# david-gimeno/tailored-avsr

Hardware: AMD Instinct MI355X
Metric: utterances/sec fwd+bwd, 12L tailored AV-Branchformer (Conv3d+ResNet-18 lip frontend, fusion, CTC+6L decoder), 4 s clips, batch 32/GPU (higher is better)
Workload: dtype f32

## Files before the change

profiles/conv_launches.py:

```python
import csv
import os
import sys
from collections import defaultdict

ROOT = os.path.dirname(os.path.dirname(os.path.abspath(__file__)))
sys.path[:0] = [ROOT, os.path.join(ROOT, "tailored-avsr_amd")]
N_IMG = 3200
LAYERS = (("layer 4", 3, 3, 512), ("layer 3", 6, 6, 256))
FLAGS = (0, 3, 1)


def labels():
    out = []
    for name, H, W, Cc in LAYERS:
        out += [f"{name} forward NT {N_IMG * H * W}x{Cc}x{9 * Cc} posmajor={f}" for f in FLAGS]
        out += [f"{name} wgrad TN {Cc}x{9 * Cc}x{N_IMG * H * W} posmajor={f}" for f in FLAGS]
    return out


def run():
    import torch
    from tavsr import ops
    for name, H, W, Cc in LAYERS:
        M, K = N_IMG * H * W, 9 * Cc
        x = torch.randn(M, Cc, device="cuda")
        w = torch.randn(Cc, K, device="cuda") / K ** 0.5
        dz = torch.randn(M, Cc, device="cuda")
        z = torch.empty(M, Cc, device="cuda")
        dw = torch.empty(Cc, K, device="cuda")
        for f in FLAGS:
            for _ in range(2):
                ops.gemm(M, Cc, K, x, Cc, w, K, z, Cc, conv=(1, H, W, Cc, 1, 9, f))
        for f in FLAGS:
            for _ in range(2):
                ops.gemm(Cc, K, M, dz, Cc, x, Cc, dw, K, a_kmajor=True, b_kmajor=True, conv=(2, H, W, Cc, 1, 9, f))
        torch.cuda.synchronize()


def summarise(path):
    rows = defaultdict(dict)
    names = {}
    with open(path) as f:
        for r in csv.DictReader(f):
            if "gemm_glds_kernel" not in r["Kernel_Name"]:
                continue
            d = int(r["Dispatch_Id"])
            rows[d][r["Counter_Name"]] = rows[d].get(r["Counter_Name"], 0.0) + float(r["Counter_Value"])
            names[d] = r["Kernel_Name"]
# ... 21 lines not shown
```

tailored-avsr_amd/csrc/gemm.hip:

```cpp
#include <algorithm>
#include <type_traits>
#include <vector>

#include <cstdlib>
#include "common.h"

namespace tavsr {

typedef float f32x16 __attribute__((ext_vector_type(16)));

struct GemmArgs {
  tavsr_gemm_desc d;
  int kchunk;
  int nsplit;
  int tiles_m, tiles_n;
  int vec_epi;
  int zmap;
};

template <int V>
__global__ __launch_bounds__(256) void splitk_epilogue_kernel(const GemmArgs args) {
  const tavsr_gemm_desc& d = args.d;
  const int64_t mn = (int64_t)d.M * d.N;
  const int nbatch = d.nb1 * d.nb2;
  const int64_t i = ((int64_t)blockIdx.x * 256 + threadIdx.x) * V;
  const int z = blockIdx.y, z1 = z / d.nb2, z2 = z % d.nb2;
  if (d.a_rowsum && z == 0 && i < d.M) {
    const float* rs = d.ws + (int64_t)args.nsplit * nbatch * mn;
    for (int q = 0; q < V && i + q < d.M; ++q) {
      float v = 0.f;
      for (int s = 0; s < args.nsplit; ++s) v += rs[(int64_t)s * d.M + i + q];
      d.a_rowsum[i + q] = d.alpha * v;
// ... 128 lines not shown
template <int ROWS, int BK, bool KMAJOR>
__device__ __forceinline__ void read_frag(const float* __restrict__ s, int row, int g, int lk, float (&f)[4]) {
  using T = Tile<ROWS, BK, KMAJOR>;
  if (KMAJOR) {
    const float* p = s + (g * 8 + 4 * lk) * T::LD + row;
#pragma unroll
    for (int j = 0; j < 4; ++j) f[j] = p[j * T::LD];
  } else {
    const float4 v = *reinterpret_cast<const float4*>(s + row * T::LD + g * 8 + 4 * lk);
    f[0] = v.x; f[1] = v.y; f[2] = v.z; f[3] = v.w;
  }
}

struct PosMajor {
  int n, H, W;
  int uni, base, rp;
  __host__ __device__ __forceinline__ void pos(int v, int& y, int& x) const {
    const int Hi = H > 2 ? H - 2 : 0, Wi = W > 2 ? W - 2 : 0, Hb = H - Hi, Wb = W - Wi;
    int u = v;
    if (u < Hi * Wi) { y = u / Wi + 1; x = u % Wi + 1; return; }
    u -= Hi * Wi;
    if (u < Hi * Wb) { y = u / Wb + 1; x = (u % Wb) ? W - 1 : 0; return; }
    u -= Hi * Wb;
    if (u < Hb * Wi) { y = (u / Wi) ? H - 1 : 0; x = u % Wi + 1; return; }
    u -= Hb * Wi;
    y = (u / Wb) ? H - 1 : 0;
    x = (u % Wb) ? W - 1 : 0;
  }
  __host__ __device__ __forceinline__ uint32_t taps(int y, int x) const {
    uint32_t mk = 0;
#pragma unroll
    for (int tap = 0; tap < 9; ++tap)
      mk |= (uint32_t)((unsigned)(y + tap / 3 - 1) < (unsigned)H && (unsigned)(x + tap % 3 - 1) < (unsigned)W) << tap;
    return mk;
  }
  __device__ __forceinline__ int row(int r) const {
    if (uni) return (r - base) * (H * W) + rp;
    const int v = r / n;
    int y, x;
    pos(v, y, x);
    return (r - v * n) * (H * W) + y * W + x;
  }
};

constexpr int kOrdRuns = 80;
struct TileOrder {
  int nruns;
  int start[kOrdRuns];
// ... 14 lines not shown
  }
  const int s = s0 + (uniform ? (j & 7) : j / tiles_n);
  nt = uniform ? (j >> 3) : j % tiles_n;
  int r = r0;
  while (r + 1 < o.nruns && o.cum[r + 1] <= s) ++r;
  mt = o.start[r] + s - o.cum[r];
}

__host__ __device__ inline int dw_tile_order(int q, int tiles_m, int tiles_n, int H, int W) {
  if (tiles_n % 9 != 0) return q;
  const int tpt = tiles_n / 9, per = tiles_m * tpt;
  const int rank = q / per, rem = q - rank * per;
  const unsigned long long taps = (H - 1) * W >= H * (W - 1) ? 0x862053714ull : 0x862071534ull;
  const int tap = (int)((taps >> (4 * rank)) & 15);
  return (rem / tpt) * tiles_n + tap * tpt + rem % tpt;
}

template <int TM, int TN, bool PM = false>
__device__ __forceinline__ void finish_tile(const tavsr_gemm_desc& d, int nsplit, f32x16 (&acc)[TM][TN],
                                            float (&asum)[TM], bool want_rowsum, int m0, int n0, int wm, int wn, int lr,
                                            int lk, int z1, int z2, int64_t coff, int zidx, const float* bias_pre = nullptr,
                                            const PosMajor* pm = nullptr) {
  if (want_rowsum) {
#pragma unroll
    for (int i = 0; i < TM; ++i) asum[i] += __shfl_xor(asum[i], 32, 64);
  }

  if (nsplit > 1) {
    const int64_t mn = (int64_t)d.M * d.N;
    const int nbatch = gridDim.y;
// ... 346 lines not shown
}

#ifdef TAVSR_GEMM_TRACE
constexpr int kTraceMax = 1 << 15;
__device__ unsigned long long g_trace[kTraceMax][6];
__device__ unsigned int g_trace_n;
#define TAVSR_TRACE_DECL unsigned long long tr_t[4], tr_c[4]; tr_t[0] = wall_clock64(); tr_t[1] = tr_t[0]; tr_c[1] = tr_c[2] = 0;
#define TAVSR_TRACE_AT(i) { tr_t[i] = wall_clock64(); tr_c[i] = __builtin_readcyclecounter(); }
#else
#define TAVSR_TRACE_DECL
#define TAVSR_TRACE_AT(i)
#endif

template <int BM, int BN, int WM, int WN, int S, bool AK, bool BKM, int KW = 1, int CONV = 0, bool PM = false>
__device__ __forceinline__ void glds_tile(const tavsr_gemm_desc& d, int kchunk, int nsplit, int tiles_n, int bid, bool vec_epi,
                                          int zidx) {
  constexpr int BK = 32, NG = BK / 8;
  static_assert(NG % KW == 0, "k-groups must divide over the wave sets");
  constexpr int NT = WM * WN * KW * 64;
  constexpr int TM = BM / WM / 32, TN = BN / WN / 32;
  using LA = GLoader<BM, AK, NT>;
  using LB = GLoader<BN, BKM, NT>;
  constexpr int ASZ = BM * BK, STAGE = (BM + BN) * BK;
  constexpr int NR4A = BM * BK / NT, NR4B = BN * BK / NT;
  constexpr int G = (CONV == 4 ? NR4A : LA::NR) + (CONV == 5 ? NR4B : LB::NR);
  static_assert((S - 2) * G <= 63, "vmcnt field");
  static_assert(!PM || (KW == 1 && ((CONV == 1 && !AK) || (CONV == 2 && AK && BKM))), "position-major order: the 3x3 convolution's GEMMs");
  __shared__ __attribute__((aligned(1024))) float smem[S * STAGE];

  const int tid = threadIdx.x;
  const int lane = tid & 63;
// ... 16 lines not shown
#pragma unroll
    for (int j = 0; j < TN; ++j)
#pragma unroll
      for (int r = 0; r < 16; ++r) acc[i][j][r] = 0.f;
  float asum[TM];
#pragma unroll
  for (int i = 0; i < TM; ++i) asum[i] = 0.f;
  const bool want_rowsum = d.a_rowsum != nullptr && n0 == (PM && CONV == 2 ? 4 * d.conv_C : 0) && wn == 0;
  float bpre[TN];
#pragma unroll
  for (int j = 0; j < TN; ++j) {
    const int n = n0 + wn * TN * 32 + j * 32 + lr;
    bpre[j] = (d.bias && nsplit == 1 && n < d.N) ? d.bias[n] : 0.f;
  }

  const int kbeg = zidx * kchunk;
  const int kend = min(d.K, kbeg + kchunk);
  int nk = CONV == 3 ? (kend - kbeg + BK - 1) / BK : (kend - kbeg) / BK;
  const int64_t kstepA = AK ? (int64_t)BK * d.lda : BK;
  const int64_t kstepB = BKM ? (int64_t)BK * d.ldb : BK;
  int64_t offA[LA::NR], offB[LB::NR];
  LA::offsets(d.lda, m0, d.M, tid, offA);
  LB::offsets(d.ldb, n0, d.N, tid, offB);
  const float* Ak = A + (AK ? (int64_t)kbeg * d.lda : kbeg);
  const float* Bk = B + (BKM ? (int64_t)kbeg * d.ldb : kbeg);
  uint32_t cmask[LA::NR];
  const int cs = d.conv_stride > 1 ? d.conv_stride : 1;
  const bool c9 = d.conv_taps != 1;
  const int cp0 = (CONV == 1 || CONV == 2) && d.conv_taps == 90 ? 1 : 0;
  const int cHo = CONV ? (d.conv_H - 1 - 2 * cp0) / cs + 1 : 1, cWo = CONV ? (d.conv_W - 1 - 2 * cp0) / cs + 1 : 1;
  PosMajor pm{};
  uint32_t pm_taps = 0;
  int pm_tap = 0, pm_cb = 0;
  if (PM && CONV == 1) {
    pm.H = d.conv_H; pm.W = d.conv_W;
    pm.n = d.M / (d.conv_H * d.conv_W);
    const int vlo = m0 / pm.n, vhi = min(m0 + BM - 1, d.M - 1) / pm.n;
    for (int v = vlo; v <= vhi; ++v) {
      int y, x;
      pm.pos(v, y, x);
      pm_taps |= pm.taps(y, x);
      pm.rp = y * d.conv_W + x;
    }
    pm.uni = vlo == vhi;
    pm.base = vlo * pm.n;
    nk = 0;
    for (int tap = 0; tap < 9; ++tap) {
      const int lo = max(kbeg, tap * d.conv_C), hi = min(kend, (tap + 1) * d.conv_C);
      if (((pm_taps >> tap) & 1u) && hi > lo) nk += (hi - lo) / BK;
    }
    pm_tap = kbeg / d.conv_C;
    pm_cb = (kbeg - pm_tap * d.conv_C) / BK;
    if (!((pm_taps >> pm_tap) & 1u)) {
      const uint32_t up = pm_taps >> (pm_tap + 1) << (pm_tap + 1);
      pm_tap = up ? __builtin_ctz(up) : 9;
      pm_cb = 0;
    }
#pragma unroll
    for (int i = 0; i < LA::NR; ++i) {
      const int q = i * NT + tid, row = q >> 3;
      const int r = min(m0 + row, d.M - 1);
      int y, x, img;
      if (pm.uni) {
        y = pm.rp / d.conv_W; x = pm.rp - y * d.conv_W; img = r - pm.base;
      } else {
        const int v = r / pm.n;
        pm.pos(v, y, x);
        img = r - v * pm.n;
      }
      offA[i] = ((int64_t)img * (d.conv_H * d.conv_W) + y * d.conv_W + x) * d.lda + ((q & 7) ^ ((row >> 1) & 7)) * 4;
      cmask[i] = pm.taps(y, x);
    }
  } else if (CONV == 1) {
#pragma unroll
    for (int i = 0; i < LA::NR; ++i) {
      const int m = min(m0 + ((i * NT + tid) >> 3), d.M - 1);
      const int x = (m % cWo) * cs + cp0, y = ((m / cWo) % cHo) * cs + cp0;
      if (cs > 1 || cp0) offA[i] += ((int64_t)((m / (cWo * cHo)) * d.conv_H + y) * d.conv_W + x - m) * d.conv_C;
      uint32_t mk = 0;
#pragma unroll
      for (int tap = 0; tap < 9; ++tap)
        mk |= (uint32_t)((unsigned)(y + tap / 3 - 1) < (unsigned)d.conv_H && (unsigned)(x + tap % 3 - 1) < (unsigned)d.conv_W) << tap;
      cmask[i] = c9 ? mk : 1u;
    }
  }
// ... 78 lines not shown
    c2_cb = n0 - tap * d.conv_C;
    c2_dy = c9 ? tap / 3 - 1 : 0;
    c2_dx = c9 ? tap % 3 - 1 : 0;
    c2_tapoff = c2_dy * d.conv_W + c2_dx;
#pragma unroll
    for (int i = 0; i < LB::NR; ++i) {
      const int m = kbeg + (i * NT + tid) / (BN / 4);
      const int t = m / cWo;
      c2_ox[i] = m - t * cWo;
      c2_img[i] = t / cHo;
      c2_oy[i] = t - c2_img[i] * cHo;
    }
  }
  int p2_n = 1, p2_i0 = 0, p2_v = 0, p2_img = 0, p2_x = 0, p2_y = 0;
  auto p2_ok = [&](int y, int x) {
    return (unsigned)(y + c2_dy) < (unsigned)d.conv_H && (unsigned)(x + c2_dx) < (unsigned)d.conv_W;
  };
  auto p2_advance = [&]() {
    p2_img += BK;
    while (p2_img >= p2_n) {
      p2_img -= p2_n;
      ++p2_v;
      if (++p2_x == d.conv_W) { p2_x = 0; ++p2_y; }
    }
  };
  if (PM && CONV == 2) {
    const int P = d.conv_H * d.conv_W;
    p2_i0 = kbeg / P;
    p2_n = (kend - kbeg) / P;
#pragma unroll
    for (int i = 0; i < LA::NR; ++i) offA[i] -= (int64_t)((i * NT + tid) / (BM / 4)) * d.lda;
    if (p2_n % BK == 0) {
      nk = (p2_n / BK) * max(d.conv_H - abs(c2_dy), 0) * max(d.conv_W - abs(c2_dx), 0);
    } else {
      nk = 0;
      int prev = 0, y = 0, x = 0;
      for (int v = 0; v < P; ++v) {
        if (p2_ok(y, x)) {
          const int s_lo = max(v * p2_n / BK, prev), s_hi = ((v + 1) * p2_n - 1) / BK + 1;
          if (s_hi > s_lo) { nk += s_hi - s_lo; prev = s_hi; }
        }
        if (++x == d.conv_W) { x = 0; ++y; }
      }
    }
  }
  int kofsA[LA::NR], kofsB[LB::NR];
  if (CONV == 3) {
#pragma unroll
    for (int i = 0; i < LA::NR; ++i) {
      const int q = i * NT + tid;
      kofsA[i] = AK ? q / (BM / 4) : ((q & 7) ^ (((q >> 3) >> 1) & 7)) * 4;
    }
#pragma unroll
    for (int i = 0; i < LB::NR; ++i) {
      const int q = i * NT + tid;
      kofsB[i] = BKM ? q / (BN / 4) : ((q & 7) ^ (((q >> 3) >> 1) & 7)) * 4;
    }
  }
  auto issue = [&](int kt, int st) {
    if (PM && CONV == 2) {
      for (;;) {
        bool any = false;
        int end = p2_img + BK, y = p2_y, x = p2_x;
        for (;;) {
          any |= p2_ok(y, x);
          if (end <= p2_n) break;
          end -= p2_n;
          if (++x == d.conv_W) { x = 0; ++y; }
        }
        if (any) break;
        p2_advance();
      }
      const int P = d.conv_H * d.conv_W;
      auto locate = [&](int kl, int& y, int& x) {
        int img = p2_img + kl, v = p2_v;
        y = p2_y; x = p2_x;
        while (img >= p2_n) {
          img -= p2_n;
          ++v;
          if (++x == d.conv_W) { x = 0; ++y; }
        }
        return (int64_t)(p2_i0 + img) * P + v;
      };
#pragma unroll
      for (int i = 0; i < LA::NR; ++i) {
        int y, x;
        const int64_t pix = locate((i * NT + tid) / (BM / 4), y, x);
        __builtin_amdgcn_global_load_lds((glb_float*)(A + pix * d.lda + offA[i]), (lds_float*)(smem + st * STAGE + (i * NT + wave * 64) * 4), 16, 0, 0);
      }
#pragma unroll
      for (int i = 0; i < LB::NR; ++i) {
        const int r = (((i * NT + tid) % (BN / 4)) * 4);
        int y, x;
        const int64_t pix = locate((i * NT + tid) / (BN / 4), y, x);
        const float* src = p2_ok(y, x) ? B + (pix + c2_tapoff) * d.conv_C + c2_cb + r : d.conv_zero;
        __builtin_amdgcn_global_load_lds((glb_float*)src, (lds_float*)(smem + st * STAGE + ASZ + (i * NT + wave * 64) * 4), 16, 0, 0);
      }
      p2_advance();
      return;
    }
    int kpm = 0, kpm_tap = 0;
    if (PM) {
      kpm_tap = pm_tap;
      kpm = pm_tap * d.conv_C + pm_cb * BK;
      const int wrap = (pm_cb + 1) * BK >= d.conv_C;
      const uint32_t up = pm_taps >> (pm_tap + 1) << (pm_tap + 1);
      pm_cb = wrap ? 0 : pm_cb + 1;
      pm_tap = !wrap ? pm_tap : up ? __builtin_ctz(up) : 9;
    }
// ... 252 lines not shown

template <int BM, int BN, int WM, int WN, int S, int MINW, bool AK, bool BKM, int KW = 1, int CONV = 0, bool PM = false>
__global__ __launch_bounds__(WM* WN * KW * 64, MINW)
void gemm_glds_kernel(const std::conditional_t<PM && CONV == 1, GemmArgsOrd, GemmArgs> xargs) {
  const GemmArgs& args = common_args(xargs);
  int bid = xcd_remap(blockIdx.x, gridDim.x), zidx = blockIdx.z;
  if constexpr (PM && CONV == 1) {
    if (xargs.ord.nruns > 0) {
      int mt, nt;
      tile_order_map(xargs.ord, blockIdx.x, args.tiles_m, args.tiles_n, mt, nt);
      bid = mt * args.tiles_n + nt;
    }
  }
  if (args.zmap) {
    const int tiles = gridDim.x, l = blockIdx.x + tiles * blockIdx.z, j = l >> 3;
    zidx = (l & 7) + 8 * (j / tiles);
    bid = j % tiles;
    if constexpr (PM && CONV == 2) {
      if (!(args.d.conv_posmajor & 2)) bid = dw_tile_order(bid, args.tiles_m, args.tiles_n, args.d.conv_H, args.d.conv_W);
    }
  }
  glds_tile<BM, BN, WM, WN, S, AK, BKM, KW, CONV, PM>(args.d, args.kchunk, args.nsplit, args.tiles_n, bid, args.vec_epi != 0, zidx);
}

constexpr int kMaxGroup = 12;
struct GroupArgs {
  tavsr_gemm_desc d[kMaxGroup];
  int tile_start[kMaxGroup + 1];
  int tiles_n[kMaxGroup];
  int n;
  int vec_epi;
};

template <int BM, int BN, int WM, int WN, int S, int MINW, bool AK, bool BKM>
__global__ __launch_bounds__(WM* WN * 64, MINW)
void gemm_glds_grouped_kernel(const GroupArgs g) {
  const int bid = xcd_remap(blockIdx.x, gridDim.x);
// ... 120 lines not shown
}

template <int BM, int BN, int WM, int WN, int S, int MINW, int KW = 1>
static int launch_glds(const tavsr_gemm_desc& d, int nsplit, int kchunk, hipStream_t s) {
  GemmArgs a{d, kchunk, nsplit, cdiv(d.M, BM), cdiv(d.N, BN), (int)vec_epi_ok(d)};
  dim3 grid(a.tiles_m * a.tiles_n, d.nb1 * d.nb2, nsplit);
  int rc = launch_layout(d, [&](auto ak, auto bk) {
    hipLaunchKernelGGL((gemm_glds_kernel<BM, BN, WM, WN, S, MINW, decltype(ak)::value, decltype(bk)::value, KW>), grid,
                       dim3(WM * WN * KW * 64), 0, s, a);
    TAVSR_LAUNCH_CHECK();
    return (int)TAVSR_OK;
  });
  return rc ? rc : launch_epilogue(a, s);
}

static bool conv_pm(const tavsr_gemm_desc& d) {
  return d.conv_posmajor && (d.conv_mode == 1 || d.conv_mode == 2) && d.conv_stride <= 1 && (d.conv_taps == 0 || d.conv_taps == 9) &&
         (d.conv_mode == 2 || !d.a_rowsum);
}

static void tile_order_build(const tavsr_gemm_desc& d, int BM, int nsplit, TileOrder& o) {
  o.nruns = 0;
  const int P = d.conv_H * d.conv_W;
  if (nsplit != 1 || (d.conv_posmajor & 2) || P <= 0 || d.M < P) return;
  struct Key { int H, W, M, BM; };
  static thread_local Key last{0, 0, 0, 0};
  static thread_local TileOrder last_o;
  if (last.H == d.conv_H && last.W == d.conv_W && last.M == d.M && last.BM == BM) { o = last_o; return; }
  PosMajor pm{};
  pm.H = d.conv_H; pm.W = d.conv_W; pm.n = d.M / P;
  std::vector<uint32_t> tp(P);
  for (int v = 0; v < P; ++v) {
    int y, x;
    pm.pos(v, y, x);
    tp[v] = pm.taps(y, x);
  }
  struct Run { int start, len, w; };
  std::vector<Run> runs;
  const int tiles_m = cdiv(d.M, BM);
  for (int i = 0; i < tiles_m; ++i) {
    const int vlo = (int)((int64_t)i * BM / pm.n);
    const int vhi = std::min((int)(std::min<int64_t>((int64_t)i * BM + BM - 1, d.M - 1) / pm.n), P - 1);
    uint32_t mk = 0;
    for (int v = vlo; v <= vhi; ++v) mk |= tp[v];
    const int w = __builtin_popcount(mk);
    if (!runs.empty() && runs.back().w == w) ++runs.back().len;
    else runs.push_back(Run{i, 1, w});
    if ((int)runs.size() > kOrdRuns) return;
  }
  std::stable_sort(runs.begin(), runs.end(), [](const Run& a, const Run& b) { return a.w > b.w; });
  int cum = 0;
  for (size_t r = 0; r < runs.size(); ++r) {
    o.start[r] = runs[r].start; o.cum[r] = cum; o.w[r] = runs[r].w;
    cum += runs[r].len;
  }
  o.cum[runs.size()] = cum;
  o.nruns = (int)runs.size();
  last = Key{d.conv_H, d.conv_W, d.M, BM};
  last_o = o;
}

static int launch_conv(const tavsr_gemm_desc& d, int nsplit, int kchunk, hipStream_t s) {
  const int ve = (int)vec_epi_ok(d);
  constexpr int wide = 1;
  constexpr int dw_wide = 1;
  constexpr int zmap_on = 1;
  const int zmap = zmap_on && (d.conv_mode == 2 || d.conv_mode == 5 || d.conv_mode == 7) && nsplit >= 8 && nsplit % 8 == 0;
  if (d.conv_mode == 6 || d.conv_mode == 7) {
    GemmArgs a6{d, kchunk, nsplit, cdiv(d.M, 64), cdiv(d.N, 64), ve, zmap};
    const dim3 grid6(a6.tiles_m * a6.tiles_n, 1, nsplit);
    constexpr int st3 = 2;
    constexpr int tile128 = 0;
    if (d.conv_mode == 6 && tile128) {
      GemmArgs a7{d, kchunk, nsplit, cdiv(d.M, 128), cdiv(d.N, 64), ve, 0};
      hipLaunchKernelGGL((gemm_glds_kernel<128, 64, 2, 2, 2, 3, false, false, 1, 6>), dim3(a7.tiles_m * a7.tiles_n, 1, 1), dim3(256), 0, s, a7);
      TAVSR_LAUNCH_CHECK();
      return TAVSR_OK;
// ... 20 lines not shown
    return launch_epilogue(a4, s);
  }
  const bool pm = conv_pm(d) && d.conv_mode == 1, pm2 = conv_pm(d) && d.conv_mode == 2;
  if (d.conv_mode == 1 && !d.b_kmajor && nsplit == 1 && wide && d.N % 128 == 0) {
    GemmArgs a2{d, kchunk, nsplit, cdiv(d.M, 64), cdiv(d.N, 128), (int)vec_epi_ok(d)};
    if (pm) {
      GemmArgsOrd ao{a2, {}};
      tile_order_build(d, 64, nsplit, ao.ord);
      hipLaunchKernelGGL((gemm_glds_kernel<64, 128, 2, 2, 2, 3, false, false, 1, 1, true>), dim3(a2.tiles_m * a2.tiles_n, 1, 1), dim3(256), 0, s, ao);
    } else
      hipLaunchKernelGGL((gemm_glds_kernel<64, 128, 2, 2, 2, 3, false, false, 1, 1>), dim3(a2.tiles_m * a2.tiles_n, 1, 1), dim3(256), 0, s, a2);
    TAVSR_LAUNCH_CHECK();
    return TAVSR_OK;
  }
  if (d.conv_mode == 2 && dw_wide && d.M % 128 == 0) {
    GemmArgs a2{d, kchunk, nsplit, cdiv(d.M, 128), cdiv(d.N, 64), (int)vec_epi_ok(d), zmap};
    if (pm2)
      hipLaunchKernelGGL((gemm_glds_kernel<128, 64, 2, 2, 2, 3, true, true, 1, 2, true>), dim3(a2.tiles_m * a2.tiles_n, 1, nsplit), dim3(256), 0, s, a2);
    else
      hipLaunchKernelGGL((gemm_glds_kernel<128, 64, 2, 2, 2, 3, true, true, 1, 2>), dim3(a2.tiles_m * a2.tiles_n, 1, nsplit), dim3(256), 0, s, a2);
    TAVSR_LAUNCH_CHECK();
    return launch_epilogue(a2, s);
  }
  GemmArgs a{d, kchunk, nsplit, cdiv(d.M, 64), cdiv(d.N, 64), ve, zmap};
  dim3 grid(a.tiles_m * a.tiles_n, 1, nsplit);
  if (pm) {
    GemmArgsOrd ao{a, {}};
    tile_order_build(d, 64, nsplit, ao.ord);
    if (!d.b_kmajor)
      hipLaunchKernelGGL((gemm_glds_kernel<64, 64, 2, 2, 2, 5, false, false, 1, 1, true>), grid, dim3(256), 0, s, ao);
    else
      hipLaunchKernelGGL((gemm_glds_kernel<64, 64, 2, 2, 2, 5, false, true, 1, 1, true>), grid, dim3(256), 0, s, ao);
  } else if (d.conv_mode == 1 && !d.b_kmajor)
    hipLaunchKernelGGL((gemm_glds_kernel<64, 64, 2, 2, 2, 5, false, false, 1, 1>), grid, dim3(256), 0, s, a);
  else if (d.conv_mode == 1)
    hipLaunchKernelGGL((gemm_glds_kernel<64, 64, 2, 2, 2, 5, false, true, 1, 1>), grid, dim3(256), 0, s, a);
  else if (pm2)
    hipLaunchKernelGGL((gemm_glds_kernel<64, 64, 2, 2, 2, 5, true, true, 1, 2, true>), grid, dim3(256), 0, s, a);
  else
// ... 34 lines not shown
    case 0: return launch_glds<128, 128, 2, 2, 3, 1>(d, nsplit, kchunk, s);
    case 1: return launch_glds<128, 128, 2, 4, 3, 2>(d, nsplit, kchunk, s);
    case 2: return launch_glds<128, 64, 2, 2, 3, 2>(d, nsplit, kchunk, s);
    case 3: return launch_glds<64, 128, 2, 2, 3, 2>(d, nsplit, kchunk, s);
    case 4: return launch_glds<64, 64, 2, 2, 3, 3>(d, nsplit, kchunk, s);
    case 5: return launch_glds<64, 64, 2, 2, 4, 2>(d, nsplit, kchunk, s);
    case 6: return launch_glds<128, 64, 2, 2, 4, 1>(d, nsplit, kchunk, s);
    case 7: return launch_glds<64, 64, 2, 2, 3, 4, 2>(d, nsplit, kchunk, s);
    case 8: return launch_glds<64, 64, 2, 2, 2, 5>(d, nsplit, kchunk, s);
    default: return launch_fallback(d, vec, nsplit, kchunk, s);
  }
}

struct Plan {
  int cfg, nsplit, kchunk;
};

static bool glds_ok(const tavsr_gemm_desc& d, bool vec) {
  return vec && d.K % 32 == 0 && d.K >= 32 && (!d.a_kmajor || d.M % 4 == 0) && (!d.b_kmajor || d.N % 4 == 0);
}

static bool tail_ok(const tavsr_gemm_desc& d, bool vec) {
  constexpr int on = 1;
  const int64_t k4 = (d.K + 3) / 4 * 4;
  return on && vec && d.K % 32 != 0 && d.K >= 32 && (!d.a_kmajor || d.M % 4 == 0) && (!d.b_kmajor || d.N % 4 == 0) &&
         (d.a_kmajor || d.lda >= k4) && (d.b_kmajor || d.ldb >= k4) && d.conv_mode == 0;
}

static Plan plan(const tavsr_gemm_desc& d, bool allow_split, bool fast) {
  const long nbatch = (long)d.nb1 * d.nb2;
// ... 2 lines not shown
  constexpr int forced = -1;
  auto variant = [&](long blocks) { (void)blocks; return !fast ? kFallbackCfg : forced >= 0 ? forced : 8; };
  p.cfg = variant(tiles);
  if (!allow_split || tiles >= 384 || d.K < 512) return p;
  if (d.K <= 1024 && tiles >= 150) return p;
  constexpr long target = 1000L;
  long want = std::min<long>((target + tiles / 2) / tiles, d.K / 256);
  if (want < 2) return p;
  p.kchunk = cdiv(cdiv(d.K, want), 32) * 32;
  p.nsplit = cdiv(d.K, p.kchunk);
  if (p.nsplit < 2) p = Plan{p.cfg, 1, d.K};
  p.cfg = variant(tiles * p.nsplit);
  return p;
}

static Plan plan_conv(const tavsr_gemm_desc& d, bool can_split) {
  Plan pc = plan(d, can_split, true);
  if ((d.conv_mode == 2 || d.conv_mode == 5 || d.conv_mode == 7) && can_split) {
    constexpr int dw_wide = 1;
    const bool wide = d.conv_mode == 2 && dw_wide && d.M % 128 == 0;
    const long tiles = (long)cdiv(d.M, wide ? 128 : 64) * cdiv(d.N, 64);
    constexpr long target64 = 2560L;
    constexpr long target128 = 2304L;
    const long target = wide ? target128 : target64;
    int unit = 32;
    if (conv_pm(d)) {
      const int P = d.conv_H * d.conv_W;
      int g = P, b = 32;
      while (b) { const int t = g % b; g = b; b = t; }
      unit = P / g * 32;
      if (pc.nsplit > 1) {
        pc.kchunk = cdiv(pc.kchunk, unit) * unit;
        pc.nsplit = cdiv(d.K, pc.kchunk);
      }
    }
    const long want = std::min<long>(std::max<long>(1, target / tiles), d.K / 512);
    if (want > pc.nsplit) {
      pc.kchunk = cdiv(cdiv(d.K, want), unit) * unit;
      pc.nsplit = cdiv(d.K, pc.kchunk);
    }
    if (pc.nsplit >= 16 && pc.nsplit % 8 != 0) {
      for (long w8 = pc.nsplit / 8 * 8; w8 >= 8; w8 -= 8) {
        const int kc = cdiv(cdiv(d.K, w8), unit) * unit;
        if (cdiv(d.K, kc) % 8 == 0) { pc.kchunk = kc; pc.nsplit = cdiv(d.K, kc); break; }
        if (w8 < pc.nsplit / 2) break;
      }
    }
  }
  return pc;
}

static bool aligned16(const void* p) { return (reinterpret_cast<uintptr_t>(p) & 15) == 0; }

static int64_t ws_floats_for(const tavsr_gemm_desc& d, int nsplit) {
  if (nsplit <= 1) return 0;
  return (int64_t)nsplit * d.nb1 * d.nb2 * d.M * d.N + (d.a_rowsum ? (int64_t)nsplit * d.M : 0);
}

__global__ __launch_bounds__(256) void ext_epilogue_kernel(const tavsr_gemm_desc d) {
  const int64_t i = ((int64_t)blockIdx.x * 256 + threadIdx.x) * 4;
// ... 104 lines not shown
    }
    const int cs = d.conv_stride > 1 ? d.conv_stride : 1, taps = d.conv_taps == 1 ? 1 : 9;
    TAVSR_REQUIRE(d.conv_taps == 0 || d.conv_taps == 1 || d.conv_taps == 9 || d.conv_taps == 90, TAVSR_EINVAL,
                  "tavsr_gemm: conv_taps must be 1, 9 or 90 (3x3 without padding)");
    const int p0 = d.conv_taps == 90 ? 1 : 0;
    TAVSR_REQUIRE(!p0 || (d.conv_H >= 3 && d.conv_W >= 3), TAVSR_EINVAL, "tavsr_gemm: an unpadded 3x3 window needs a 3x3 image");
    const int64_t pixels = d.conv_mode == 1 ? d.M : d.K;
    const int64_t per_image = (int64_t)((d.conv_H - 1 - 2 * p0) / cs + 1) * ((d.conv_W - 1 - 2 * p0) / cs + 1);
    TAVSR_REQUIRE(pixels % per_image == 0, TAVSR_EINVAL, "tavsr_gemm: conv rows are not whole images");
    if (d.conv_mode == 1)
      TAVSR_REQUIRE(!d.a_kmajor && d.K == taps * d.conv_C && d.conv_C % 32 == 0 && d.lda == d.conv_C, TAVSR_EUNSUPPORTED,
                    "tavsr_gemm: conv mode 1 needs a row-major image operand A, K = taps * C, C %% 32 == 0");
    else
      TAVSR_REQUIRE(d.a_kmajor && d.b_kmajor && d.N == taps * d.conv_C && d.conv_C % 64 == 0 && d.ldb == d.conv_C,
                    TAVSR_EUNSUPPORTED, "tavsr_gemm: conv mode 2 needs the TN layout, N = taps * C, C %% 64 == 0");
    Plan pc = plan_conv(d, can_split);
    if (pc.nsplit > 1 && d.ws_floats < ws_floats_for(d, pc.nsplit)) pc = plan(d, false, true);
    return launch_conv(d, pc.nsplit, pc.kchunk, s);
  }
  const bool tail = !fast && force_cfg < 0 && tail_ok(d, vec);
  if (d.drop_p > 0.f) {
    TAVSR_REQUIRE(d.drop_p < 1.f && d.drop_seed && d.drop_offset % 4 == 0, TAVSR_EINVAL,
                  "tavsr_gemm: dropout needs p in (0, 1), a device seed and an offset %% 4 == 0");
    TAVSR_REQUIRE((fast || tail) && force_cfg < 0 && d.nb1 * d.nb2 == 1 && vec_epi_ok(d), TAVSR_EUNSUPPORTED,
                  "tavsr_gemm: epilogue dropout needs an unbatched problem on the 16-byte path");
  }
  TAVSR_REQUIRE((d.rowdot_a == nullptr) == (d.rowdot_b == nullptr) && (!d.rowdot_a || d.rowstat), TAVSR_EINVAL,
                "tavsr_gemm: rowdot_a and rowdot_b go together, with rowstat as their output");
  if (d.rowstat) {
    TAVSR_REQUIRE(fast && force_cfg < 0 && d.nb1 * d.nb2 == 1 && vec_epi_ok(d) && aligned16(d.rowstat) && aligned16(d.rowdot_a) &&
                      aligned16(d.rowdot_b), TAVSR_EUNSUPPORTED,
                  "tavsr_gemm: row statistics / row dots need an unbatched problem on the 16-byte path");
    return launch(8, d, vec, 1, d.K, s);
// ... 104 lines not shown
  d.conv_H = H; d.conv_W = W; d.M = images * H * W; d.conv_posmajor = 1;
  TileOrder o;
  tile_order_build(d, bm, 1, o);
  if (o.nruns == 0) return 0;
  const int tiles_m = cdiv(d.M, bm), nwg = tiles_m * tiles_n;
  for (int b = 0; b < nwg && b < max_blocks; ++b) tile_order_map(o, b, tiles_m, tiles_n, tile_m[b], tile_n[b]);
  return nwg;
}

extern "C" int tavsr_conv_dw_tile_order(int H, int W, int tiles_m, int tiles_n, int32_t* tile, int max_tiles) {
  if (H <= 0 || W <= 0 || tiles_m <= 0 || tiles_n <= 0) return 0;
  for (int q = 0; q < tiles_m * tiles_n && q < max_tiles; ++q) tile[q] = tavsr::dw_tile_order(q, tiles_m, tiles_n, H, W);
  return tiles_m * tiles_n;
}

#ifdef TAVSR_GEMM_TRACE
extern "C" int tavsr_gemm_trace_read(unsigned long long* out, int max_rows) {
  unsigned int n = 0;
  if (hipDeviceSynchronize() != hipSuccess) return -1;
  if (hipMemcpyFromSymbol(&n, HIP_SYMBOL(tavsr::g_trace_n), sizeof(n)) != hipSuccess) return -1;
  int rows = (int)(n < (unsigned)tavsr::kTraceMax ? n : tavsr::kTraceMax);
  if (rows > max_rows) rows = max_rows;
  if (rows > 0 && hipMemcpyFromSymbol(out, HIP_SYMBOL(tavsr::g_trace), (size_t)rows * 6 * sizeof(unsigned long long)) != hipSuccess) return -1;
  n = 0;
  if (hipMemcpyToSymbol(HIP_SYMBOL(tavsr::g_trace_n), &n, sizeof(n)) != hipSuccess) return -1;
  return rows;
}
#endif
```

tailored-avsr_amd/tavsr/ops.py:

```python
from __future__ import annotations

import ctypes as C
import os
from typing import Optional, Sequence

import torch

from . import _lib as L
from ._lib import ACT, AttnDesc, GemmDesc, check, lib, ptr, require_cuda, stream

f32 = torch.float32


def empty(*shape, like: Optional[torch.Tensor] = None, dtype=f32, device=None):
    dev = like.device if like is not None else (device if device is not None else "cuda")
    return torch.empty(shape, dtype=dtype, device=dev)


_addr = L.addr


class GemmProfile:

    def __init__(self, by_shape: bool = False):
# ... 1439 lines not shown

def avgpool_bwd(dy, N, P, Cn):
    dx = empty(N * P, Cn, like=dy)
    check(lib().tavsr_avgpool_bwd(ptr(dy), ptr(dx), N, P, Cn, stream()), "tavsr_avgpool_bwd")
    return dx


def conv_wflip(w2d, cout, cin):
    require_cuda(w2d)
    out = empty(cin, 9 * cout, like=w2d)
    check(lib().tavsr_conv_wflip(ptr(w2d), ptr(out), cout, cin, stream()), "tavsr_conv_wflip")
    return out


CONV_TAPSKIP = os.environ.get("TAVSR_CONV_TAPSKIP", "1") != "0"
CONV_TAPSKIP_MAXPOS = int(os.environ.get("TAVSR_CONV_TAPSKIP_MAXPOS", "36"))
CONV_TILEORDER = os.environ.get("TAVSR_CONV_TILEORDER", "1") != "0"


def _tapskip(H, W, stride=1, taps=9, pad0=False):
    on = CONV_TAPSKIP and stride == 1 and taps == 9 and not pad0 and H * W <= CONV_TAPSKIP_MAXPOS
    return (1 if CONV_TILEORDER else 3) if on else 0


def conv3x3_fwd(x, w2d, H, W, stride=1, taps=9, pad0=False, bias=None, act=None):
    M, cin = x.shape
    cout = w2d.shape[0]
    if pad0:
        assert taps == 9
        Ho, Wo = (H - 3) // stride + 1, (W - 3) // stride + 1
    else:
        Ho, Wo = (H - 1) // stride + 1, (W - 1) // stride + 1
    Mo = M // (H * W) * Ho * Wo
    z = empty(Mo, cout, like=x)
    gemm(Mo, cout, taps * cin, x, cin, w2d, taps * cin, z, cout, conv=(1, H, W, cin, stride, 90 if pad0 else taps, _tapskip(H, W, stride, taps, pad0)),
         bias=bias, act=act)
    return z


def conv3x3_dx(dz, wflip, H, W, res=None):
    M, cout = dz.shape
    cin = wflip.shape[0]
    dx = empty(M, cin, like=dz)
    gemm(M, cin, 9 * cout, dz, cout, wflip, 9 * cout, dx, cin, conv=(1, H, W, cout, 0, 0, _tapskip(H, W)), R=res, ldr=0 if res is None else cin)
    return dx


def conv3x3_dw(dz, x, H, W, stride=1, taps=9, pad0=False, bias_grad=False):
    M, cout = dz.shape
    cin = x.shape[1]
    dw = empty(cout, taps * cin, like=dz)
    gb = empty(cout, like=dz) if bias_grad else None
    gemm(cout, taps * cin, M, dz, cout, x, cin, dw, taps * cin, a_kmajor=True, b_kmajor=True,
         conv=(2, H, W, cin, stride, 90 if pad0 else taps, _tapskip(H, W, stride, taps, pad0)), a_rowsum=gb)
    return (dw, gb) if bias_grad else dw


def fill_(t, value):
    require_cuda(t)
    assert t.is_contiguous()
    check(lib().tavsr_fill(ptr(t), value, t.numel(), stream()), "tavsr_fill")
    return t


def copy2d(src, dst):
    require_cuda(src, dst)
    assert src.shape == dst.shape and src.dim() == 2 and src.stride(1) == 1 and dst.stride(1) == 1
    check(lib().tavsr_copy2d(ptr(src), src.stride(0), ptr(dst), dst.stride(0), src.shape[0], src.shape[1], stream()), "tavsr_copy2d")
    return dst
# ... 417 lines not shown
```

Measured before the change: 408.1.

## Extend position-major tap-skip conv to stride-2 and larger maps; uneven dW split-K

Generalises the position-major tap-skipping implicit-GEMM conv path to stride-2 convolutions by tracking output vs input dims and strides, and raises the default forward/dx tap-skip position limit from 36 to 121. For weight-gradient convs it adds an uneven split-K plan, where the first n_big slices take one extra unit, plus an XCD-aware slice/tile ordering so the split count can hit the occupancy target. The aim is to skip zero-padded taps on more layers and balance split-K work. In exchange it adds indexing complexity and risks slower paths on larger maps where tap skipping saves little.

```diff
diff --git a/profiles/conv_launches.py b/profiles/conv_launches.py
--- a/profiles/conv_launches.py
+++ b/profiles/conv_launches.py
@@ -8,13 +8,14 @@
 N_IMG = 3200
 LAYERS = (("layer 4", 3, 3, 512), ("layer 3", 6, 6, 256))
 FLAGS = (0, 3, 1)
+DW_FLAGS = (0, 3, 1, 5)
 
 
 def labels():
     out = []
     for name, H, W, Cc in LAYERS:
         out += [f"{name} forward NT {N_IMG * H * W}x{Cc}x{9 * Cc} posmajor={f}" for f in FLAGS]
-        out += [f"{name} wgrad TN {Cc}x{9 * Cc}x{N_IMG * H * W} posmajor={f}" for f in FLAGS]
+        out += [f"{name} wgrad TN {Cc}x{9 * Cc}x{N_IMG * H * W} posmajor={f}" for f in DW_FLAGS]
     return out
 
 
@@ -31,7 +32,7 @@
         for f in FLAGS:
             for _ in range(2):
                 ops.gemm(M, Cc, K, x, Cc, w, K, z, Cc, conv=(1, H, W, Cc, 1, 9, f))
-        for f in FLAGS:
+        for f in DW_FLAGS:
             for _ in range(2):
                 ops.gemm(Cc, K, M, dz, Cc, x, Cc, dw, K, a_kmajor=True, b_kmajor=True, conv=(2, H, W, Cc, 1, 9, f))
         torch.cuda.synchronize()
diff --git a/profiles/dump_outputs_cmp.py b/profiles/dump_outputs_cmp.py
--- /dev/null
+++ b/profiles/dump_outputs_cmp.py
@@ -0,0 +1,24 @@
+import os
+import sys
+
+import numpy as np
+
+a_dir, b_dir = sys.argv[1], sys.argv[2]
+names = open(sys.argv[3]).read().split() if len(sys.argv) > 3 and os.path.exists(sys.argv[3]) else None
+for f in sorted(os.listdir(a_dir)):
+    if not f.endswith(".npy"):
+        continue
+    a, b = np.load(os.path.join(a_dir, f)).ravel(), np.load(os.path.join(b_dir, f)).ravel()
+    assert a.shape == b.shape, (f, a.shape, b.shape)
+    diff = np.flatnonzero(a.view(np.uint32 if a.dtype == np.float32 else np.uint64) != b.view(np.uint32 if b.dtype == np.float32 else np.uint64))
+    key = f[:-4]
+    if diff.size == 0:
+        print(f"{key}: bit-identical ({a.size} entries)")
+        continue
+    rel = np.abs(a[diff].astype(np.float64) - b[diff]) / np.maximum(np.abs(a[diff].astype(np.float64)), 1e-300)
+    print(f"{key}: {diff.size} of {a.size} entries differ, max rel {rel.max():.3e}")
+    if diff.size <= 64:
+        print(f"  parameter indices: {diff.tolist()}")
+        if names and key == "grad_norm":
+            print(f"  names: {[names[i] for i in diff]}")
+        print(f"  rel: {[f'{r:.2e}' for r in rel]}")
diff --git a/tailored-avsr_amd/csrc/gemm.hip b/tailored-avsr_amd/csrc/gemm.hip
--- a/tailored-avsr_amd/csrc/gemm.hip
+++ b/tailored-avsr_amd/csrc/gemm.hip
@@ -16,6 +16,7 @@
   int tiles_m, tiles_n;
   int vec_epi;
   int zmap;
+  int n_big, kunit;
 };
 
 template <int V>
@@ -174,6 +175,7 @@
 
 struct PosMajor {
   int n, H, W;
+  int st, HI, WI;
   int uni, base, rp;
   __host__ __device__ __forceinline__ void pos(int v, int& y, int& x) const {
     const int Hi = H > 2 ? H - 2 : 0, Wi = W > 2 ? W - 2 : 0, Hb = H - Hi, Wb = W - Wi;
@@ -191,7 +193,7 @@
     uint32_t mk = 0;
 #pragma unroll
     for (int tap = 0; tap < 9; ++tap)
-      mk |= (uint32_t)((unsigned)(y + tap / 3 - 1) < (unsigned)H && (unsigned)(x + tap % 3 - 1) < (unsigned)W) << tap;
+      mk |= (uint32_t)((unsigned)(st * y + tap / 3 - 1) < (unsigned)HI && (unsigned)(st * x + tap % 3 - 1) < (unsigned)WI) << tap;
     return mk;
   }
   __device__ __forceinline__ int row(int r) const {
@@ -236,6 +238,17 @@
   const unsigned long long taps = (H - 1) * W >= H * (W - 1) ? 0x862053714ull : 0x862071534ull;
   const int tap = (int)((taps >> (4 * rank)) & 15);
   return (rem / tpt) * tiles_n + tap * tpt + rem % tpt;
+}
+
+__host__ __device__ inline void dw_xcd_order(int j, int tiles_m, int tiles_n, int ns, int& zs, int& q) {
+  const int tiles = tiles_m * tiles_n;
+  zs = j / tiles;
+  q = j - zs * tiles;
+  if (tiles_n % 9 != 0) return;
+  const int per = tiles_m * (tiles_n / 9);
+  const int rank = j / (ns * per), rem = j - rank * (ns * per);
+  zs = rem / per;
+  q = rank * per + rem - zs * per;
 }
 
 template <int TM, int TN, bool PM = false>
@@ -612,7 +625,7 @@
 
 template <int BM, int BN, int WM, int WN, int S, bool AK, bool BKM, int KW = 1, int CONV = 0, bool PM = false>
 __device__ __forceinline__ void glds_tile(const tavsr_gemm_desc& d, int kchunk, int nsplit, int tiles_n, int bid, bool vec_epi,
-                                          int zidx) {
+                                          int zidx, int n_big = 0, int kunit = 0) {
   constexpr int BK = 32, NG = BK / 8;
   static_assert(NG % KW == 0, "k-groups must divide over the wave sets");
   constexpr int NT = WM * WN * KW * 64;
@@ -659,8 +672,8 @@
     bpre[j] = (d.bias && nsplit == 1 && n < d.N) ? d.bias[n] : 0.f;
   }
 
-  const int kbeg = zidx * kchunk;
-  const int kend = min(d.K, kbeg + kchunk);
+  const int kbeg = zidx * kchunk + min(zidx, n_big) * kunit;
+  const int kend = min(d.K, kbeg + kchunk + (zidx < n_big ? kunit : 0));
   int nk = CONV == 3 ? (kend - kbeg + BK - 1) / BK : (kend - kbeg) / BK;
   const int64_t kstepA = AK ? (int64_t)BK * d.lda : BK;
   const int64_t kstepB = BKM ? (int64_t)BK * d.ldb : BK;
@@ -678,14 +691,15 @@
   uint32_t pm_taps = 0;
   int pm_tap = 0, pm_cb = 0;
   if (PM && CONV == 1) {
-    pm.H = d.conv_H; pm.W = d.conv_W;
-    pm.n = d.M / (d.conv_H * d.conv_W);
+    pm.H = cHo; pm.W = cWo;
+    pm.st = cs; pm.HI = d.conv_H; pm.WI = d.conv_W;
+    pm.n = d.M / (cHo * cWo);
     const int vlo = m0 / pm.n, vhi = min(m0 + BM - 1, d.M - 1) / pm.n;
     for (int v = vlo; v <= vhi; ++v) {
       int y, x;
       pm.pos(v, y, x);
       pm_taps |= pm.taps(y, x);
-      pm.rp = y * d.conv_W + x;
+      pm.rp = y * cWo + x;
     }
     pm.uni = vlo == vhi;
     pm.base = vlo * pm.n;
@@ -707,13 +721,13 @@
       const int r = min(m0 + row, d.M - 1);
       int y, x, img;
       if (pm.uni) {
-        y = pm.rp / d.conv_W; x = pm.rp - y * d.conv_W; img = r - pm.base;
+        y = pm.rp / cWo; x = pm.rp - y * cWo; img = r - pm.base;
       } else {
         const int v = r / pm.n;
         pm.pos(v, y, x);
         img = r - v * pm.n;
       }
-      offA[i] = ((int64_t)img * (d.conv_H * d.conv_W) + y * d.conv_W + x) * d.lda + ((q & 7) ^ ((row >> 1) & 7)) * 4;
+      offA[i] = ((int64_t)img * (d.conv_H * d.conv_W) + cs * y * d.conv_W + cs * x) * d.lda + ((q & 7) ^ ((row >> 1) & 7)) * 4;
       cmask[i] = pm.taps(y, x);
     }
   } else if (CONV == 1) {
@@ -822,24 +836,27 @@
   }
   int p2_n = 1, p2_i0 = 0, p2_v = 0, p2_img = 0, p2_x = 0, p2_y = 0;
   auto p2_ok = [&](int y, int x) {
-    return (unsigned)(y + c2_dy) < (unsigned)d.conv_H && (unsigned)(x + c2_dx) < (unsigned)d.conv_W;
+    return (unsigned)(cs * y + c2_dy) < (unsigned)d.conv_H && (unsigned)(cs * x + c2_dx) < (unsigned)d.conv_W;
   };
   auto p2_advance = [&]() {
     p2_img += BK;
     while (p2_img >= p2_n) {
       p2_img -= p2_n;
       ++p2_v;
-      if (++p2_x == d.conv_W) { p2_x = 0; ++p2_y; }
+      if (++p2_x == cWo) { p2_x = 0; ++p2_y; }
     }
   };
   if (PM && CONV == 2) {
-    const int P = d.conv_H * d.conv_W;
+    const int P = cHo * cWo;
     p2_i0 = kbeg / P;
     p2_n = (kend - kbeg) / P;
 #pragma unroll
     for (int i = 0; i < LA::NR; ++i) offA[i] -= (int64_t)((i * NT + tid) / (BM / 4)) * d.lda;
     if (p2_n % BK == 0) {
-      nk = (p2_n / BK) * max(d.conv_H - abs(c2_dy), 0) * max(d.conv_W - abs(c2_dx), 0);
+      int ny = 0, nx = 0;
+      for (int y = 0; y < cHo; ++y) ny += (unsigned)(cs * y + c2_dy) < (unsigned)d.conv_H;
+      for (int x = 0; x < cWo; ++x) nx += (unsigned)(cs * x + c2_dx) < (unsigned)d.conv_W;
+      nk = (p2_n / BK) * ny * nx;
     } else {
       nk = 0;
       int prev = 0, y = 0, x = 0;
@@ -848,7 +865,7 @@
           const int s_lo = max(v * p2_n / BK, prev), s_hi = ((v + 1) * p2_n - 1) / BK + 1;
           if (s_hi > s_lo) { nk += s_hi - s_lo; prev = s_hi; }
         }
-        if (++x == d.conv_W) { x = 0; ++y; }
+        if (++x == cWo) { x = 0; ++y; }
       }
     }
   }
@@ -874,33 +891,36 @@
           any |= p2_ok(y, x);
           if (end <= p2_n) break;
           end -= p2_n;
-          if (++x == d.conv_W) { x = 0; ++y; }
+          if (++x == cWo) { x = 0; ++y; }
         }
         if (any) break;
         p2_advance();
       }
-      const int P = d.conv_H * d.conv_W;
-      auto locate = [&](int kl, int& y, int& x) {
-        int img = p2_img + kl, v = p2_v;
+      const int P = cHo * cWo;
+      auto locate = [&](int kl, int& y, int& x, int& img) {
+        int v = p2_v;
+        img = p2_img + kl;
         y = p2_y; x = p2_x;
         while (img >= p2_n) {
           img -= p2_n;
           ++v;
-          if (++x == d.conv_W) { x = 0; ++y; }
+          if (++x == cWo) { x = 0; ++y; }
         }
-        return (int64_t)(p2_i0 + img) * P + v;
+        img += p2_i0;
+        return (int64_t)img * P + v;
       };
 #pragma unroll
       for (int i = 0; i < LA::NR; ++i) {
-        int y, x;
-        const int64_t pix = locate((i * NT + tid) / (BM / 4), y, x);
+        int y, x, img;
+        const int64_t pix = locate((i * NT + tid) / (BM / 4), y, x, img);
         __builtin_amdgcn_global_load_lds((glb_float*)(A + pix * d.lda + offA[i]), (lds_float*)(smem + st * STAGE + (i * NT + wave * 64) * 4), 16, 0, 0);
       }
 #pragma unroll
       for (int i = 0; i < LB::NR; ++i) {
         const int r = (((i * NT + tid) % (BN / 4)) * 4);
-        int y, x;
-        const int64_t pix = locate((i * NT + tid) / (BN / 4), y, x);
+        int y, x, img;
+        locate((i * NT + tid) / (BN / 4), y, x, img);
+        const int64_t pix = ((int64_t)img * d.conv_H + cs * y) * d.conv_W + cs * x;
         const float* src = p2_ok(y, x) ? B + (pix + c2_tapoff) * d.conv_C + c2_cb + r : d.conv_zero;
         __builtin_amdgcn_global_load_lds((glb_float*)src, (lds_float*)(smem + st * STAGE + ASZ + (i * NT + wave * 64) * 4), 16, 0, 0);
       }
@@ -1183,13 +1203,18 @@
   }
   if (args.zmap) {
     const int tiles = gridDim.x, l = blockIdx.x + tiles * blockIdx.z, j = l >> 3;
-    zidx = (l & 7) + 8 * (j / tiles);
+    int zs = j / tiles;
     bid = j % tiles;
     if constexpr (PM && CONV == 2) {
-      if (!(args.d.conv_posmajor & 2)) bid = dw_tile_order(bid, args.tiles_m, args.tiles_n, args.d.conv_H, args.d.conv_W);
-    }
-  }
-  glds_tile<BM, BN, WM, WN, S, AK, BKM, KW, CONV, PM>(args.d, args.kchunk, args.nsplit, args.tiles_n, bid, args.vec_epi != 0, zidx);
+      if (!(args.d.conv_posmajor & 2)) {
+        if (args.n_big > 0) dw_xcd_order(j, args.tiles_m, args.tiles_n, args.nsplit >> 3, zs, bid);
+        bid = dw_tile_order(bid, args.tiles_m, args.tiles_n, args.d.conv_H, args.d.conv_W);
+      }
+    }
+    zidx = (l & 7) + 8 * zs;
+  }
+  glds_tile<BM, BN, WM, WN, S, AK, BKM, KW, CONV, PM>(args.d, args.kchunk, args.nsplit, args.tiles_n, bid, args.vec_epi != 0, zidx,
+                                                      args.n_big, args.kunit);
 }
 
 constexpr int kMaxGroup = 12;
@@ -1340,21 +1365,28 @@
   return rc ? rc : launch_epilogue(a, s);
 }
 
+static int conv_ho(const tavsr_gemm_desc& d) { return (d.conv_H - 1) / std::max(d.conv_stride, 1) + 1; }
+static int conv_wo(const tavsr_gemm_desc& d) { return (d.conv_W - 1) / std::max(d.conv_stride, 1) + 1; }
+
+constexpr int kPmStride2MaxPos = 36;
 static bool conv_pm(const tavsr_gemm_desc& d) {
-  return d.conv_posmajor && (d.conv_mode == 1 || d.conv_mode == 2) && d.conv_stride <= 1 && (d.conv_taps == 0 || d.conv_taps == 9) &&
+  const bool stride_ok = d.conv_stride <= 1 || (d.conv_stride == 2 && (d.conv_posmajor & 8) && conv_ho(d) * conv_wo(d) <= kPmStride2MaxPos);
+  return d.conv_posmajor && (d.conv_mode == 1 || d.conv_mode == 2) && stride_ok && (d.conv_taps == 0 || d.conv_taps == 9) &&
          (d.conv_mode == 2 || !d.a_rowsum);
 }
 
 static void tile_order_build(const tavsr_gemm_desc& d, int BM, int nsplit, TileOrder& o) {
   o.nruns = 0;
-  const int P = d.conv_H * d.conv_W;
+  const int cs = std::max(d.conv_stride, 1);
+  const int P = conv_ho(d) * conv_wo(d);
   if (nsplit != 1 || (d.conv_posmajor & 2) || P <= 0 || d.M < P) return;
-  struct Key { int H, W, M, BM; };
-  static thread_local Key last{0, 0, 0, 0};
+  struct Key { int H, W, cs, M, BM; };
+  static thread_local Key last{0, 0, 0, 0, 0};
   static thread_local TileOrder last_o;
-  if (last.H == d.conv_H && last.W == d.conv_W && last.M == d.M && last.BM == BM) { o = last_o; return; }
+  if (last.H == d.conv_H && last.W == d.conv_W && last.cs == cs && last.M == d.M && last.BM == BM) { o = last_o; return; }
   PosMajor pm{};
-  pm.H = d.conv_H; pm.W = d.conv_W; pm.n = d.M / P;
+  pm.H = conv_ho(d); pm.W = conv_wo(d); pm.n = d.M / P;
+  pm.st = cs; pm.HI = d.conv_H; pm.WI = d.conv_W;
   std::vector<uint32_t> tp(P);
   for (int v = 0; v < P; ++v) {
     int y, x;
@@ -1382,11 +1414,11 @@
   }
   o.cum[runs.size()] = cum;
   o.nruns = (int)runs.size();
-  last = Key{d.conv_H, d.conv_W, d.M, BM};
+  last = Key{d.conv_H, d.conv_W, cs, d.M, BM};
   last_o = o;
 }
 
-static int launch_conv(const tavsr_gemm_desc& d, int nsplit, int kchunk, hipStream_t s) {
+static int launch_conv(const tavsr_gemm_desc& d, int nsplit, int kchunk, hipStream_t s, int n_big = 0, int kunit = 0) {
   const int ve = (int)vec_epi_ok(d);
   constexpr int wide = 1;
   constexpr int dw_wide = 1;
@@ -1437,7 +1469,7 @@
     return TAVSR_OK;
   }
   if (d.conv_mode == 2 && dw_wide && d.M % 128 == 0) {
-    GemmArgs a2{d, kchunk, nsplit, cdiv(d.M, 128), cdiv(d.N, 64), (int)vec_epi_ok(d), zmap};
+    GemmArgs a2{d, kchunk, nsplit, cdiv(d.M, 128), cdiv(d.N, 64), (int)vec_epi_ok(d), zmap, pm2 ? n_big : 0, pm2 ? kunit : 0};
     if (pm2)
       hipLaunchKernelGGL((gemm_glds_kernel<128, 64, 2, 2, 2, 3, true, true, 1, 2, true>), dim3(a2.tiles_m * a2.tiles_n, 1, nsplit), dim3(256), 0, s, a2);
     else
@@ -1445,7 +1477,7 @@
     TAVSR_LAUNCH_CHECK();
     return launch_epilogue(a2, s);
   }
-  GemmArgs a{d, kchunk, nsplit, cdiv(d.M, 64), cdiv(d.N, 64), ve, zmap};
+  GemmArgs a{d, kchunk, nsplit, cdiv(d.M, 64), cdiv(d.N, 64), ve, zmap, pm2 ? n_big : 0, pm2 ? kunit : 0};
   dim3 grid(a.tiles_m * a.tiles_n, 1, nsplit);
   if (pm) {
     GemmArgsOrd ao{a, {}};
@@ -1510,6 +1542,7 @@
 
 struct Plan {
   int cfg, nsplit, kchunk;
+  int n_big = 0, kunit = 0;
 };
 
 static bool glds_ok(const tavsr_gemm_desc& d, bool vec) {
@@ -1542,7 +1575,7 @@
   return p;
 }
 
-static Plan plan_conv(const tavsr_gemm_desc& d, bool can_split) {
+static Plan plan_conv(const tavsr_gemm_desc& d, bool can_split, int force_split = 0) {
   Plan pc = plan(d, can_split, true);
   if ((d.conv_mode == 2 || d.conv_mode == 5 || d.conv_mode == 7) && can_split) {
     constexpr int dw_wide = 1;
@@ -1553,7 +1586,7 @@
     const long target = wide ? target128 : target64;
     int unit = 32;
     if (conv_pm(d)) {
-      const int P = d.conv_H * d.conv_W;
+      const int P = conv_ho(d) * conv_wo(d);
       int g = P, b = 32;
       while (b) { const int t = g % b; g = b; b = t; }
       unit = P / g * 32;
@@ -1572,6 +1605,17 @@
         const int kc = cdiv(cdiv(d.K, w8), unit) * unit;
         if (cdiv(d.K, kc) % 8 == 0) { pc.kchunk = kc; pc.nsplit = cdiv(d.K, kc); break; }
         if (w8 < pc.nsplit / 2) break;
+      }
+    }
+    if (conv_pm(d) && d.conv_mode == 2 && !(d.conv_posmajor & 4) && d.K % unit == 0) {
+      const long U = d.K / unit, round4 = (wide ? 768 : 1280) / 4;
+      const long w = std::min<long>(force_split > 0 ? force_split : want, U) / 8 * 8;
+      const bool missed = target - (long)pc.nsplit * tiles > round4, hits = target - w * tiles <= round4;
+      if (w >= 8 && U % w != 0 && (force_split > 0 || (missed && hits))) {
+        pc.nsplit = (int)w;
+        pc.kchunk = (int)(U / w) * unit;
+        pc.n_big = (int)(U % w);
+        pc.kunit = unit;
       }
     }
   }
@@ -1706,9 +1750,9 @@
     else
       TAVSR_REQUIRE(d.a_kmajor && d.b_kmajor && d.N == taps * d.conv_C && d.conv_C % 64 == 0 && d.ldb == d.conv_C,
                     TAVSR_EUNSUPPORTED, "tavsr_gemm: conv mode 2 needs the TN layout, N = taps * C, C %% 64 == 0");
-    Plan pc = plan_conv(d, can_split);
+    Plan pc = plan_conv(d, can_split, force_split);
     if (pc.nsplit > 1 && d.ws_floats < ws_floats_for(d, pc.nsplit)) pc = plan(d, false, true);
-    return launch_conv(d, pc.nsplit, pc.kchunk, s);
+    return launch_conv(d, pc.nsplit, pc.kchunk, s, pc.n_big, pc.kunit);
   }
   const bool tail = !fast && force_cfg < 0 && tail_ok(d, vec);
   if (d.drop_p > 0.f) {
@@ -1843,6 +1887,28 @@
   return tiles_m * tiles_n;
 }
 
+extern "C" int tavsr_conv_dw_plan(int H, int W, int cin, int cout, int images, int posmajor, int force_split, int32_t* out) {
+  using namespace tavsr;
+  if (H <= 0 || W <= 0 || cin <= 0 || cout <= 0 || images <= 0 || !out) return 0;
+  tavsr_gemm_desc d{};
+  d.conv_mode = 2; d.conv_H = H; d.conv_W = W; d.conv_C = cin; d.conv_stride = 1; d.conv_taps = 9; d.conv_posmajor = posmajor;
+  d.M = cout; d.N = 9 * cin; d.K = images * H * W; d.a_kmajor = d.b_kmajor = 1; d.nb1 = d.nb2 = 1;
+  const Plan p = plan_conv(d, true, force_split);
+  out[0] = p.kchunk; out[1] = p.n_big; out[2] = p.kunit;
+  return p.nsplit;
+}
+
+extern "C" int tavsr_conv_dw_xcd_order(int H, int W, int tiles_m, int tiles_n, int ns, int32_t* slice, int32_t* tile, int max_tiles) {
+  if (H <= 0 || W <= 0 || tiles_m <= 0 || tiles_n <= 0 || ns <= 0) return 0;
+  for (int j = 0; j < ns * tiles_m * tiles_n && j < max_tiles; ++j) {
+    int zs, q;
+    tavsr::dw_xcd_order(j, tiles_m, tiles_n, ns, zs, q);
+    slice[j] = zs;
+    tile[j] = tavsr::dw_tile_order(q, tiles_m, tiles_n, H, W);
+  }
+  return ns * tiles_m * tiles_n;
+}
+
 #ifdef TAVSR_GEMM_TRACE
 extern "C" int tavsr_gemm_trace_read(unsigned long long* out, int max_rows) {
   unsigned int n = 0;
diff --git a/tailored-avsr_amd/tavsr/ops.py b/tailored-avsr_amd/tavsr/ops.py
--- a/tailored-avsr_amd/tavsr/ops.py
+++ b/tailored-avsr_amd/tavsr/ops.py
@@ -1477,13 +1477,33 @@
 
 
 CONV_TAPSKIP = os.environ.get("TAVSR_CONV_TAPSKIP", "1") != "0"
-CONV_TAPSKIP_MAXPOS = int(os.environ.get("TAVSR_CONV_TAPSKIP_MAXPOS", "36"))
+CONV_TAPSKIP_MAXPOS = int(os.environ.get("TAVSR_CONV_TAPSKIP_MAXPOS", "121"))
 CONV_TILEORDER = os.environ.get("TAVSR_CONV_TILEORDER", "1") != "0"
-
-
-def _tapskip(H, W, stride=1, taps=9, pad0=False):
-    on = CONV_TAPSKIP and stride == 1 and taps == 9 and not pad0 and H * W <= CONV_TAPSKIP_MAXPOS
-    return (1 if CONV_TILEORDER else 3) if on else 0
+CONV_TAPSKIP_MAXPOS_DW = int(os.environ.get("TAVSR_CONV_TAPSKIP_MAXPOS_DW", "36"))
+CONV_DW_UNEVEN = os.environ.get("TAVSR_CONV_DW_UNEVEN", "1") != "0"
+
+
+CONV_TAPSKIP_STRIDE2 = os.environ.get("TAVSR_CONV_TAPSKIP_STRIDE2", "1") != "0"
+CONV_TAPSKIP_STRIDE2_DW = os.environ.get("TAVSR_CONV_TAPSKIP_STRIDE2_DW", "0") != "0"
+CONV_TAPSKIP_STRIDE2_MAXPOS = 36
+
+
+def _tapskip_bits():
+    return 1 | (0 if CONV_TILEORDER else 2) | (0 if CONV_DW_UNEVEN else 4)
+
+
+def _tapskip(H, W, stride=1, taps=9, pad0=False, dw=False):
+    on = CONV_TAPSKIP and stride == 1 and taps == 9 and not pad0 and H * W <= (CONV_TAPSKIP_MAXPOS_DW if dw else CONV_TAPSKIP_MAXPOS)
+    return _tapskip_bits() if on else 0
+
+
+def _tapskip2(H, W, dw=False):
+    on = CONV_TAPSKIP and (CONV_TAPSKIP_STRIDE2_DW if dw else CONV_TAPSKIP_STRIDE2)
+    return (_tapskip_bits() | 8) if on and ((H - 1) // 2 + 1) * ((W - 1) // 2 + 1) <= CONV_TAPSKIP_STRIDE2_MAXPOS else 0
+
+
+def _tapskip_any(H, W, stride, taps, pad0, dw=False):
+    return _tapskip2(H, W, dw) if stride == 2 and taps == 9 and not pad0 else _tapskip(H, W, stride, taps, pad0, dw)
 
 
 def conv3x3_fwd(x, w2d, H, W, stride=1, taps=9, pad0=False, bias=None, act=None):
@@ -1496,7 +1516,7 @@
         Ho, Wo = (H - 1) // stride + 1, (W - 1) // stride + 1
     Mo = M // (H * W) * Ho * Wo
     z = empty(Mo, cout, like=x)
-    gemm(Mo, cout, taps * cin, x, cin, w2d, taps * cin, z, cout, conv=(1, H, W, cin, stride, 90 if pad0 else taps, _tapskip(H, W, stride, taps, pad0)),
+    gemm(Mo, cout, taps * cin, x, cin, w2d, taps * cin, z, cout, conv=(1, H, W, cin, stride, 90 if pad0 else taps, _tapskip_any(H, W, stride, taps, pad0)),
          bias=bias, act=act)
     return z
 
@@ -1509,13 +1529,13 @@
     return dx
 
 
-def conv3x3_dw(dz, x, H, W, stride=1, taps=9, pad0=False, bias_grad=False):
+def conv3x3_dw(dz, x, H, W, stride=1, taps=9, pad0=False, bias_grad=False, force=None):
     M, cout = dz.shape
     cin = x.shape[1]
     dw = empty(cout, taps * cin, like=dz)
     gb = empty(cout, like=dz) if bias_grad else None
     gemm(cout, taps * cin, M, dz, cout, x, cin, dw, taps * cin, a_kmajor=True, b_kmajor=True,
-         conv=(2, H, W, cin, stride, 90 if pad0 else taps, _tapskip(H, W, stride, taps, pad0)), a_rowsum=gb)
+         conv=(2, H, W, cin, stride, 90 if pad0 else taps, _tapskip_any(H, W, stride, taps, pad0, dw=True)), a_rowsum=gb, force=force)
     return (dw, gb) if bias_grad else dw
 
 
```

New measurement: 412.3, median of 6. 1.01x the previous value.
